# pyprob/pyprob

Hardware: NVIDIA H100
Metric: ic_train_traces_per_sec (higher is better)
Workload: dtype f32

## Files before the change

### pyprob_b200/csrc/net_tc.inc

```
extern unsigned long long* g_trace;
extern int g_trace_launch;

namespace {

inline int64_t img_floats(int64_t rows, int64_t cols) {
  return ((rows + 127) / 128) * ((cols + 31) / 32) * tc::kTileFloats;
}

__global__ void __launch_bounds__(256) k_pack_table(const float* __restrict__ arena, const PackEntry* __restrict__ tab,
                                                     int n_entries, float* __restrict__ wimg) {
  int tile = blockIdx.x;
  int lo = 0, hi = n_entries - 1;
  while (lo < hi) {
    int mid = (lo + hi + 1) >> 1;
    if (tab[mid].tile_start <= tile) lo = mid; else hi = mid - 1;
  }
  const PackEntry e = tab[lo];
  const int rt = tile - e.tile_start;
  const float* src = arena + e.src_off;
  for (int q = threadIdx.x + blockIdx.y * blockDim.x; q < 128 * e.kb * 8; q += blockDim.x * gridDim.y) {
    int c16 = q & 7, t = q >> 3;
    int cb = t % e.kb, r = t / e.kb;
    int row = rt * 128 + r, k0 = cb * 32 + c16 * 4;
    float h[4], l[4];
// ... 65 lines not shown
    gemm::Phase& ph = phases.back();
    if (p.M <= 0 || p.N <= 0 || p.K <= 0) return;
    p.tiles_m = (p.M + 127) / 128;
    p.tiles_n = (p.N + 127) / 128;
    p.tile_start = ph.tiles;
    if (p.k_splits < 1) p.k_splits = 1;
    ph.tiles += p.tiles_m * p.tiles_n * p.k_splits;
    ph.count += 1;
    probs.push_back(p);
  }
};

inline tcg::Operand op_k(const float* hi, const float* lo, int kb, int row0, int col0) {
  tcg::Operand o; o.hi = hi; o.lo = lo; o.k_rows = nullptr; o.kb = kb; o.mn = 0; o.row0 = row0; o.col0 = col0; return o;
}
inline tcg::Operand op_mn(const float* hi, const float* lo, int kb, int row0, int col0, const int* k_rows = nullptr) {
  tcg::Operand o; o.hi = hi; o.lo = lo; o.k_rows = k_rows; o.kb = kb; o.mn = 1; o.row0 = row0; o.col0 = col0; return o;
}
inline tcg::Problem TP0() { tcg::Problem p; memset(&p, 0, sizeof(p)); return p; }
inline tcg::Operand wk(const ppb_net* net, const WImg& w) { return op_k(net->wimg + w.k_hi, net->wimg + w.k_lo, w.kb, 0, 0); }
inline tcg::Operand wmn(const ppb_net* net, const WImg& w) { return op_mn(net->wimg + w.mn_hi, net->wimg + w.mn_lo, w.kb, 0, 0); }

template <bool X3, int EPI>
int launch_tc(const gemm::Phase& ph, const tcg::Problem* dev, cudaStream_t st, unsigned long long* tr) {
  static bool attr_set = false;
  if (!attr_set) {
    PPB_CUDA(cudaFuncSetAttribute(tcg::k_grouped<X3, EPI>, cudaFuncAttributeMaxDynamicSharedMemorySize, (int)tcg::smem_bytes()));
    attr_set = true;
  }
  if (ppb_persistent_enabled() && ph.tiles > PPB_NUM_SMS && tr == nullptr) {
    static bool attr_p = false;
    if (!attr_p) {
      PPB_CUDA(cudaFuncSetAttribute(tcp::k_grouped_persistent<X3, EPI>, cudaFuncAttributeMaxDynamicSharedMemorySize,
                                    (int)tcp::smem_bytes()));
      attr_p = true;
    }
    PPB_CUDA(ppb_launch(tcp::k_grouped_persistent<X3, EPI>, dim3(PPB_NUM_SMS), dim3(tcg::kThreads), tcp::smem_bytes(), st, 1, 0,
                        dev + ph.first, ph.count, ph.tiles));
    return PPB_OK;
  }
  PPB_CUDA(ppb_launch(tcg::k_grouped<X3, EPI>, dim3((unsigned)ph.tiles), dim3(tcg::kThreads), tcg::smem_bytes(), st, 1, 0,
                      dev + ph.first, ph.count, tr));
  return PPB_OK;
}

int run_tc_phase(const gemm::Phase& ph, const tcg::Problem* dev, int precision, cudaStream_t st, int epi,
                 const TcBuilder* bl_for_prof = nullptr) {
  if (ph.count == 0) return PPB_OK;
  cudaEvent_t e0;
  int rc2 = prof_begin(bl_for_prof != nullptr, st, e0); if (rc2) return rc2;
  unsigned long long* tr = nullptr;
  if (g_trace && g_trace_launch < 256) { tr = g_trace + 16 * g_trace_launch; ++g_trace_launch; }
  const bool x3 = precision == PPB_PREC_TF32X3;
  if (epi == 0) rc2 = x3 ? launch_tc<true, 0>(ph, dev, st, tr) : launch_tc<false, 0>(ph, dev, st, tr);
  else if (epi == 1) rc2 = x3 ? launch_tc<true, 1>(ph, dev, st, tr) : launch_tc<false, 1>(ph, dev, st, tr);
  else rc2 = x3 ? launch_tc<true, 2>(ph, dev, st, tr) : launch_tc<false, 2>(ph, dev, st, tr);
  if (rc2) return rc2;
  PPB_LAUNCH_CHECK();
  return e0 ? prof_end(e0, st, phase_flops(bl_for_prof->probs, ph)) : PPB_OK;
}

inline int pick_cluster(int tiles, int min_kc, bool spread_epilogue = false) {
  int cs = 1;
  while (cs < 8 && tiles * cs * 2 <= PPB_NUM_SMS && (spread_epilogue || min_kc / (cs * 2) >= 2)) cs *= 2;
  return cs;
}

template <bool X3, int CS, int EPI, typename RE = tcc::NoRowEpi>
int launch_cluster_tc(const gemm::Phase& ph, const tcg::Problem* dev, cudaStream_t st, const RE& re = RE()) {
  static bool attr_set = false;
  if (!attr_set) {
    PPB_CUDA(cudaFuncSetAttribute(tcc::k_cluster<X3, CS, EPI, RE>, cudaFuncAttributeMaxDynamicSharedMemorySize,
                                  (int)tcc::smem_bytes()));
    attr_set = true;
  }
  unsigned long long* tr = nullptr;
  if (g_trace && g_trace_launch < 256) { tr = g_trace + 16 * g_trace_launch; ++g_trace_launch; }
  PPB_CUDA(tcc::launch_cluster(tcc::k_cluster<X3, CS, EPI, RE>, ph.tiles * CS, CS, tcc::smem_bytes(), st, dev + ph.first,
                               ph.count, tr, re));
// ... 284 lines not shown

int check_tc(const ppb_net* net, const ppb_batch* b) {
  PPB_CHECK_ARG(b->row_align == 128, "the tensor-core path needs a batch encoded with row_align = 128");
  PPB_CHECK_ARG(net->wimg != nullptr, "weight images not built (ppb_net_set_tables)");
  PPB_CHECK_ARG(net->desc.lstm_dim % 32 == 0, "tensor-core path: lstm_dim must be a multiple of 32");
  PPB_CHECK_ARG(b->step_addr_host && b->step_row0_host && b->step_nrows_host && b->step_t_host && b->step_prev_row0_host,
                "missing per-step host arrays");
  return PPB_OK;
}

void add_head_fwd(TcBuilder& tb, const ppb_net* net, const float* arena, const ppb_batch* b, const Ws& w, const TcWs& t,
                  const HImg& x, int kx, const int* x_row0, int& ph_h1, int& ph_h2) {
  const int NS = b->n_steps, dhkb = (net->dh_pad + 31) / 32;
  ph_h1 = (int)tb.phases.size();
  tb.begin();
  for (int s = 0; s < NS; ++s) {
    int aid = b->step_addr_host[s];
    const ppb_addr_desc& a = net->addrs[aid];
    tcg::Problem p = TP0();
    p.a = op_k(x.k_hi, x.k_lo, (int)x.kb, x_row0[s], 0);
    p.b = wk(net, net->w1[aid]);
    p.M = pad128(b->step_nrows_host[s]); p.N = a.head_hidden; p.K = kx;
    p.m_valid = b->step_nrows_host[s];
    p.flags = tcg::kRelu | tcg::kZeroInvalid;
    p.bias = arena + a.b1_off;
    p.o_k_hi = t.hid.k_hi; p.o_k_lo = t.hid.k_lo; p.o_mn_hi = t.hid.mn_hi; p.o_mn_lo = t.hid.mn_lo;
    p.o_kb = dhkb; p.o_row0 = b->step_row0_host[s]; p.o_col0 = 0;
    tb.add(p);
  }
  ph_h2 = (int)tb.phases.size();
  tb.begin();
  for (int s = 0; s < NS; ++s) {
    int aid = b->step_addr_host[s];
    const ppb_addr_desc& a = net->addrs[aid];
    tcg::Problem p = TP0();
    p.a = op_k(t.hid.k_hi, t.hid.k_lo, dhkb, b->step_row0_host[s], 0);
    p.b = wk(net, net->w2[aid]);
    p.M = pad128(b->step_nrows_host[s]); p.N = a.head_out; p.K = a.head_hidden;
    p.bias = arena + a.b2_off;
    p.c = w.out_raw + (int64_t)b->step_row0_host[s] * net->out_pad; p.ldc = net->out_pad;
    p.o_row0 = b->step_row0_host[s];
    tb.add(p);
  }
}

int run_head_nll(ppb_net* net, const ppb_batch* b, const Ws& w, const TcWs& t, const TcBuilder& tb, int ph_h2, int precision,
                 float* loss_out, int32_t* status_out, float* row_lp_out, int want_grad, cudaStream_t st) {
  Dims d = dims_of(b);
  NllArgs na;
  na.addrs = net->d_addrs; na.row_step = b->row_step; na.step_addr = b->step_addr;
  na.values = b->values; na.prior0 = b->prior0; na.prior1 = b->prior1; na.row_trace = b->row_trace;
  na.K = net->desc.mixture_k; na.inv_batch = 1.0f / (float)d.B;
  na.row_lp = row_lp_out ? row_lp_out : w.row_lp; na.d_out = want_grad ? w.d_out : nullptr; na.out_pad = net->out_pad;
  na.dimg = want_grad ? t.d_out : HImg();
  int out_max = 0;
  for (int s = 0; s < d.NS; ++s) out_max = net->addrs[b->step_addr_host[s]].head_out > out_max ? net->addrs[b->step_addr_host[s]].head_out : out_max;
  const int cs_h2 = phase_cluster(tb.phases[ph_h2], tb, true);
  if (cs_h2 > 1 && out_max <= 128) {
    NllRowEpi re;
    re.A = na; re.loss_acc = w.loss_acc; re.loss_out = loss_out; re.status_out = status_out;
    return run_tc_phase_cluster<3>(cs_h2, tb.phases[ph_h2], t.probs, precision, st, re);
  }
  int rc = run_tc_phase_auto(tb.phases[ph_h2], t.probs, precision, st, 0, tb); if (rc) return rc;
  PPB_CUDA(ppb_launch(k_head_nll, dim3(ew_grid((int64_t)d.R * 32, 256)), dim3(256), 0, st, 1, 0, (const float*)w.out_raw, na, d.R,
                      w.loss_acc, loss_out, status_out));
  PPB_LAUNCH_CHECK();
  return PPB_OK;
}

void add_head_dhid(TcBuilder& tb, const ppb_net* net, const ppb_batch* b, const Ws& w, const TcWs& t) {
  const int dhkb = (net->dh_pad + 31) / 32, okb = (net->out_pad + 31) / 32;
  tb.begin();
  for (int s = 0; s < b->n_steps; ++s) {
    int aid = b->step_addr_host[s];
    const ppb_addr_desc& a = net->addrs[aid];
    tcg::Problem p = TP0();
    p.a = op_k(t.d_out.k_hi, t.d_out.k_lo, okb, b->step_row0_host[s], 0);
    p.b = wmn(net, net->w2[aid]);
    p.M = pad128(b->step_nrows_host[s]); p.N = a.head_hidden; p.K = a.head_out;
    p.flags = tcg::kMaskImg;
    p.mask_hi = t.hid.k_hi;
    p.c = w.d_hid + (int64_t)b->step_row0_host[s] * net->dh_pad; p.ldc = net->dh_pad;
    p.o_k_hi = t.d_hid.k_hi; p.o_k_lo = t.d_hid.k_lo; p.o_mn_hi = t.d_hid.mn_hi; p.o_mn_lo = t.d_hid.mn_lo;
    p.o_kb = dhkb; p.o_row0 = b->step_row0_host[s]; p.o_col0 = 0;
    tb.add(p);
  }
}

struct HeadChunks {
  std::vector<std::vector<int>> rows;
  std::vector<int> off, x_off;
};
HeadChunks head_chunks(const ppb_net* net, const ppb_batch* b, const int* x_row0, TcBuilder& tb) {
  HeadChunks h;
  const size_t na = net->addrs.size();
  h.rows.assign(na, std::vector<int>());
  std::vector<std::vector<int>> xr(na);
  for (int s = 0; s < b->n_steps; ++s) {
    int r0 = b->step_row0_host[s], np = pad128(b->step_nrows_host[s]);
    for (int q = 0; q < np; q += 32) {
      h.rows[b->step_addr_host[s]].push_back(r0 + q);
      if (x_row0) xr[b->step_addr_host[s]].push_back(x_row0[s] + q);
    }
// ... 63 lines not shown

int tc_loss_forward(ppb_net* net, const float* arena, const ppb_batch* b, void* workspace, int precision,
                    float* loss_out, int32_t* status_out, float* row_lp_out, int want_grad, cudaStream_t st) {
  int rc = check_tc(net, b);
  if (rc) return rc;
  const ppb_net_desc& D = net->desc;
  Dims d = dims_of(b);
  Ws w = carve(net, d, workspace);
  TcWs t = carve_tc(net, d, (char*)workspace + simt_region_bytes(net, d));
  const int H = D.lstm_dim, H4 = 4 * H, E = D.obs_dim, S = D.sample_dim, I = net->I;
  const int C2 = 2 * (D.type_dim + D.addr_dim);

  TcBuilder tb;
  ObsStep os;
  rc = obs_plan_fwd(net, arena, b, w, t.obs, t.obs_emb, tb, os, st);
  if (rc) return rc;
  const int ph_pobs = (int)tb.phases.size();
  tb.begin();
  {
    tcg::Problem p = TP0();
    p.a = op_k(t.obs_emb.k_hi, t.obs_emb.k_lo, (int)t.obs_emb.kb, 0, 0);
    p.b = wk(net, net->w_ihE);
    p.M = d.B; p.N = H4; p.K = E;
    p.c = w.p_obs; p.ldc = H4;
    tb.add(p);
  }
  std::vector<int> ph_rec(d.T, -1);
  {
    int st0 = 0;
    for (int tt = 0; tt < d.T; ++tt) {
      int st1 = st0;
      while (st1 < d.NS && b->step_t_host[st1] == tt) ++st1;
      if (tt > 0) {
        ph_rec[tt] = (int)tb.phases.size();
        tb.begin();
        for (int s = st0; s < st1; ++s) {
          tcg::Problem p = TP0();
          p.a = op_k(t.h.k_hi, t.h.k_lo, (int)t.h.kb, b->step_prev_row0_host[s], 0);
          p.b = wk(net, net->w_hh);
          p.M = pad128(b->step_nrows_host[s]); p.N = H4; p.K = H;
          p.c = w.gates + (int64_t)b->step_row0_host[s] * H4; p.ldc = H4;
          tb.add(p);
        }
      }
      st0 = st1;
    }
// ... 64 lines not shown
  rc = stream_after(net, st, s2); if (rc) return rc;
  PPB_CUDA(cudaMemsetAsync(w.loss_acc, 0, 256, s1));
  k_pack_table<<<dim3(d.T > 1 ? net->pack_tiles : net->pack_tiles_no_hh, 8), 256, 0, s2>>>(arena, net->d_pack,
                                                                                         (int)net->pack.size(), net->wimg);
  PPB_LAUNCH_CHECK();
  if (fused_cell) {
    tcl::k_pack_whh_interleaved<<<dim3(H / 32, 8), 256, 0, s2>>>(arena + D.w_hh_off, H, net->whh_il,
                                                                 net->whh_il + net->whh_il_floats);
    PPB_LAUNCH_CHECK();
  }
  k_step_embed<<<ew_grid((int64_t)d.NS * C2), 256, 0, s1>>>(arena, net->d_addrs, net->d_type_off, b->step_addr,
                                                            b->step_prev_addr, d.NS, D.type_dim, D.addr_dim, w.emb_cat);
  PPB_LAUNCH_CHECK();
  k_pstep_fwd<<<ew_grid((int64_t)d.NS * H4 * 32), 256, 0, s1>>>(w.emb_cat, arena + D.w_ih_off, arena + D.b_ih_off,
                                                                arena + D.b_hh_off, d.NS, H4, I, E + S, C2, w.p_step);
  PPB_LAUNCH_CHECK();
  if (d.T > 1) {
    k_wsmp_transpose<<<ew_grid(S * H4), 256, 0, s1>>>(arena + D.w_ih_off, I, E, S, H4, w.w_smp_t);
    PPB_LAUNCH_CHECK();
    k_smp_embed<<<ew_grid((int64_t)d.R * S), 256, 0, s1>>>(arena, net->d_addrs, b->row_step, b->step_prev_addr,
                                                           b->row_prev, b->values, d.R, S, w.smp_emb);
    PPB_LAUNCH_CHECK();
  }
  rc = obs_fwd(net, arena, b, w, t.obs, t.obs_emb, tb, t.probs, os, precision, st, s2); if (rc) return rc;
  rc = run_tc_phase_auto(tb.phases[ph_pobs], t.probs, precision, st, 0, tb, true); if (rc) return rc;
  rc = stream_after(net, s1, st); if (rc) return rc;
  for (int tt = 0; tt < d.T; ++tt) {
    int r0 = b->row_off_host[tt], n = b->row_off_host[tt + 1] - r0;
    if (tt > 0 && fused_cell) {
      if (lphase[tt].count == 0) continue;
      const tcl::Step* dsteps = (const tcl::Step*)net->d_lstm_steps;
      const bool x3 = precision == PPB_PREC_TF32X3;
      const int cs = pick_cluster(lphase[tt].tiles, H / 32);
      cudaEvent_t e0;
      rc = prof_begin(true, st, e0); if (rc) return rc;
      if (cs >= 4) rc = x3 ? launch_lstm_cluster<true, 4>(lphase[tt], dsteps, S, st) : launch_lstm_cluster<false, 4>(lphase[tt], dsteps, S, st);
      else if (cs == 2) rc = x3 ? launch_lstm_cluster<true, 2>(lphase[tt], dsteps, S, st) : launch_lstm_cluster<false, 2>(lphase[tt], dsteps, S, st);
      else rc = x3 ? launch_lstm_step<true>(lphase[tt], dsteps, st) : launch_lstm_step<false>(lphase[tt], dsteps, st);
      if (rc) return rc;
      PPB_LAUNCH_CHECK();
      rc = prof_end(e0, st, 2.0 * (double)lphase[tt].tiles * 128.0 * 128.0 * H); if (rc) return rc;
      continue;
    }
    if (tt > 0) { rc = run_tc_phase(tb.phases[ph_rec[tt]], t.probs, precision, st, 0, &tb); if (rc) return rc; }
    PPB_CUDA(ppb_launch(k_cell_fwd, dim3(ew_grid((int64_t)n * H)), dim3(256), 0, st, 1, 0, w.gates, w.p_obs, w.p_step, w.w_smp_t, w.smp_emb, b->row_step,
                                                       b->row_prev, b->row_trace, w.c, w.h, t.h, r0, n, H, S, tt));
// ... 28 lines not shown
  std::vector<int> hh_a, hh_b;
  for (int s = 0; s < d.NS; ++s) {
    int r0 = b->step_row0_host[s], np = pad128(b->step_nrows_host[s]);
    for (int q = 0; q < np; q += 32)
      if (b->step_t_host[s] > 0) { hh_a.push_back(r0 + q); hh_b.push_back(b->step_prev_row0_host[s] + q); }
  }
  const int hh_a_off = (int)tb.ints.size();
  tb.ints.insert(tb.ints.end(), hh_a.begin(), hh_a.end());
  const int hh_b_off = (int)tb.ints.size();
  tb.ints.insert(tb.ints.end(), hh_b.begin(), hh_b.end());
  PPB_CHECK_ARG((int64_t)tb.ints.size() <= t.max_ints, "chunk list overflow");

  const int ph_dhid = 0;
  add_head_dhid(tb, net, b, w, t);
  const int ph_hw = (int)tb.phases.size();
  tb.begin();
  for (int s = 0; s < d.NS; ++s) {
    int aid = b->step_addr_host[s];
    const ppb_addr_desc& a = net->addrs[aid];
    tcg::Problem p = TP0();
    p.a = op_k(t.d_hid.k_hi, t.d_hid.k_lo, dhkb, b->step_row0_host[s], 0);
    p.b = wmn(net, net->w1[aid]);
    p.M = pad128(b->step_nrows_host[s]); p.N = H; p.K = a.head_hidden;
    p.c = w.dh + (int64_t)b->step_row0_host[s] * H; p.ldc = H;
    p.o_row0 = b->step_row0_host[s];
    tb.add(p);
  }
  const int ph_headw = (int)tb.phases.size();
  add_head_weight_grads(tb, net, grad, t, hc, t.h, H);
  std::vector<int> ph_rec(d.T, -1);
  {
    int st1 = d.NS;
    for (int tt = d.T - 1; tt >= 1; --tt) {
      int st0 = st1;
      while (st0 > 0 && b->step_t_host[st0 - 1] == tt) --st0;
      ph_rec[tt] = (int)tb.phases.size();
      tb.begin();
      for (int s = st0; s < st1; ++s) {
        tcg::Problem p = TP0();
        p.a = op_k(t.dgates.k_hi, t.dgates.k_lo, gkb, b->step_row0_host[s], 0);
        p.b = wmn(net, net->w_hh);
        p.M = pad128(b->step_nrows_host[s]); p.N = H; p.K = H4;
        p.c = w.dh_rec + (int64_t)b->step_prev_row0_host[s] * H; p.ldc = H;
        tb.add(p);
      }
      {
// ... 16 lines not shown
  const int ph_lstm_w = (int)tb.phases.size();
  tb.begin();
  if (!hh_a.empty()) {
    tcg::Problem p = TP0();
    p.a = op_mn(t.dgates.mn_hi, t.dgates.mn_lo, gkb, 0, 0, t.ints + hh_a_off);
    p.b = op_mn(t.h.mn_hi, t.h.mn_lo, hkb, 0, 0, t.ints + hh_b_off);
    p.M = H4; p.N = H; p.K = 32 * (int)hh_a.size();
    p.c = grad + D.w_hh_off; p.ldc = H; p.flags = tcg::kAccumulate;
    p.k_splits = pick_splits(p.M, p.N, p.K);
    tb.add(p);
  }
  {
    tcg::Problem p = TP0();
    p.a = op_mn(t.dpobs.mn_hi, t.dpobs.mn_lo, gkb, 0, 0);
    p.b = op_mn(t.obs_emb.mn_hi, t.obs_emb.mn_lo, (int)t.obs_emb.kb, 0, 0);
    p.M = H4; p.N = E; p.K = pad128(d.B);
    p.c = grad + D.w_ih_off; p.ldc = I; p.flags = tcg::kAccumulate;
    p.k_splits = pick_splits(p.M, p.N, p.K);
    tb.add(p);
    tcg::Problem q = TP0();
    q.a = op_k(t.dpobs.k_hi, t.dpobs.k_lo, gkb, 0, 0);
    q.b = wmn(net, net->w_ihE);
    q.M = d.B; q.N = E; q.K = H4;
    q.c = w.d_obs_emb; q.ldc = E;
    q.k_splits = pick_splits(q.M, q.N, q.K);
    tb.add(q);
  }
  ObsStep os;
  rc = obs_plan_bwd(net, arena, grad, b, w, t.obs, tb, os, st);
  if (rc) return rc;
  PPB_CHECK_ARG((int64_t)tb.probs.size() <= t.max_probs / 2, "tensor-core problem list overflow");
  tcg::Problem* tprobs = t.probs + t.max_probs / 2;
  rc = upload_cached(net, 3, tb.probs.data(), tb.probs.size() * sizeof(tcg::Problem), tprobs, st);
  if (rc) return rc;
  rc = upload_cached(net, 4, tb.ints.data(), tb.ints.size() * sizeof(int), t.ints, st);
  if (rc) return rc;

  cudaStream_t s1 = net->side[0], s2 = net->side[1];
  if (d.T > 1) PPB_CUDA(cudaMemsetAsync(w.dh_rec, 0, (size_t)b->row_off_host[d.T - 1] * H * sizeof(float), st));
  PPB_CUDA(cudaMemsetAsync(w.d_pstep, 0, (size_t)((const char*)(w.d_obs_emb + (int64_t)d.B * E) - (const char*)w.d_pstep), st));
  rc = run_tc_phase_auto(tb.phases[ph_dhid], tprobs, precision, st, 2, tb); if (rc) return rc;
  const bool dpobs_fused = (d.B & 127) == 0 && t.dgates.k_hi != nullptr;
  bool dpobs_packed = false;
  const int cs_cell = (d.T == 1 && dpobs_fused) ? phase_cluster(tb.phases[ph_hw], tb, true) : 1;
  if (cs_cell > 1) {
    CellBwdT1Epi re;
    re.gates = w.gates; re.c = w.c; re.row_trace = b->row_trace; re.dgates = dgates; re.pimg = t.dpobs; re.H = H;
    rc = run_tc_phase_cluster<4>(cs_cell, tb.phases[ph_hw], tprobs, precision, st, re); if (rc) return rc;
    dpobs_packed = true;
  } else {
    rc = run_tc_phase_auto(tb.phases[ph_hw], tprobs, precision, st, 0, tb); if (rc) return rc;
    const HImg gimg = d.T > 1 ? t.dgates : HImg();
    float* const dc = d.T > 1 ? w.dc : nullptr;
    for (int tt = d.T - 1; tt >= 0; --tt) {
      int r0 = b->row_off_host[tt], n = b->row_off_host[tt + 1] - r0;
      if (tt + 1 < d.T) { rc = run_tc_phase(tb.phases[ph_rec[tt + 1]], tprobs, precision, st, 1, &tb); if (rc) return rc; }
      if (tt == 0 && dpobs_fused) {
        PPB_CUDA(ppb_launch(k_cell_bwd<true>, dim3(ew_grid((int64_t)n * H)), dim3(256), 0, st, 1, 0, w.gates, w.c, w.dh, w.dh_rec,
                            dc, dgates, w.d_pobs, b->row_prev, b->row_next, b->row_trace, gimg, r0, n, H, tt, t.dpobs));
        dpobs_packed = true;
      } else {
        PPB_CUDA(ppb_launch(k_cell_bwd<false>, dim3(ew_grid((int64_t)n * H)), dim3(256), 0, st, 1, 0, w.gates, w.c, w.dh, w.dh_rec,
                            dc, dgates, w.d_pobs, b->row_prev, b->row_next, b->row_trace, gimg, r0, n, H, tt, HImg()));
      }
      PPB_LAUNCH_CHECK();
    }
  }
  rc = stream_after(net, st, s1); if (rc) return rc;
  rc = run_tc_phase(tb.phases[ph_headw], tprobs, precision, s1, 1); if (rc) return rc;
  rc = launch_head_bias_grad(net, b, w, grad, s1); if (rc) return rc;
  rc = stream_after(net, st, s2); if (rc) return rc;
  const bool one_pass = S <= 4 && H4 <= 2048;
  int max_rows = 0;
  for (int s = 0; s < d.NS; ++s) max_rows = b->step_nrows_host[s] > max_rows ? b->step_nrows_host[s] : max_rows;
  if (one_pass) {
    int slab = (d.R + 2 * PPB_NUM_SMS - 1) / (2 * PPB_NUM_SMS);
    slab = slab < 4 ? 4 : (slab > kRedSlab ? kRedSlab : slab);
    const dim3 g((max_rows + slab - 1) / slab, d.NS);
    const float* wt = d.T > 1 ? w.w_smp_t : w.p_step;
    if (H4 <= 1024)
      k_dgates_reduce<4><<<g, 256, 0, s2>>>(dgates, wt, w.smp_emb, b->values, b->step_prev_addr, b->step_row0, b->step_nrows,
                                            b->row_prev, net->d_addrs, H4, S, I, E, w.d_pstep, grad, D.w_ih_off, slab);
    else
      k_dgates_reduce<8><<<g, 256, 0, s2>>>(dgates, wt, w.smp_emb, b->values, b->step_prev_addr, b->step_row0, b->step_nrows,
                                            b->row_prev, net->d_addrs, H4, S, I, E, w.d_pstep, grad, D.w_ih_off, slab);
    PPB_LAUNCH_CHECK();
  } else {
    dim3 g((H4 + 31) / 32, d.NS);
    k_step_colsum<<<g, 256, 0, s2>>>(dgates, b->step_row0, b->step_nrows, H4, w.d_pstep);
    PPB_LAUNCH_CHECK();
  }
  {
// ... 33 lines not shown
```

### pyprob_b200/csrc/tc_cluster.cuh

```cuda
#pragma once
#include "tc_grouped.cuh"
#include "tc_lstm.cuh"

namespace tcc {

using namespace tc;

constexpr int kPitch = 128;
constexpr int kPartFloats = 128 * kPitch;
static_assert(kPartFloats * 4 <= 2 * tcg::kStages * kTileBytes, "partial tile must fit in the A stages");

__device__ __forceinline__ uint32_t cluster_ctarank() {
  uint32_t r;
  asm volatile("mov.u32 %0, %%cluster_ctarank;" : "=r"(r));
  return r;
}
__device__ __forceinline__ void cluster_sync_all() {
  asm volatile("barrier.cluster.arrive.release.aligned;" ::: "memory");
  asm volatile("barrier.cluster.wait.acquire.aligned;" ::: "memory");
}
__device__ __forceinline__ uint32_t map_to_rank(uint32_t local_smem_addr, uint32_t rank) {
  uint32_t ra;
  asm volatile("mapa.shared::cluster.u32 %0, %1, %2;" : "=r"(ra) : "r"(local_smem_addr), "r"(rank));
  return ra;
// ... 4 lines not shown
  return v;
}

struct __align__(1024) Smem {
  float a_hi[tcg::kStages][kTileFloats];
  float a_lo[tcg::kStages][kTileFloats];
  float b_hi[tcg::kStages][kTileFloats];
  float b_lo[tcg::kStages][kTileFloats];
  uint64_t full[tcg::kStages];
  uint64_t empty[tcg::kStages];
  union { tcg::Problem prob; tcl::Step step; };
};
inline size_t smem_bytes() { return sizeof(Smem) + 1024; }

#define TCC_TRACE(slot)                                                                                   \
  do {                                                                                                    \
    if (trace && blockIdx.x == 0) {                                                                       \
      unsigned long long _t;                                                                              \
      asm volatile("mov.u64 %0, %%globaltimer;" : "=l"(_t));                                              \
      trace[slot] = _t;                                                                                   \
    }                                                                                                     \
  } while (0)

template <bool X3>
__device__ __forceinline__ void mainloop_and_park(Smem& sm, const tcg::Operand& A, const tcg::Operand& B, int mt, int nt,
                                                  int c0, int c1, int warp, int lane,
                                                  unsigned long long* trace = nullptr, int b_prefetched = 0) {
  const tcg::Ring R{sm.a_hi[0], sm.a_lo[0], sm.b_hi[0], sm.b_lo[0], kTileFloats, tcg::kStages, sm.full, sm.empty};
  if (warp == tcg::kProducerWarp) {
    if (lane == 0) {
      const uint32_t bytes = (tcg::stage_bytes(A, mt) + tcg::stage_bytes(B, nt)) * (X3 ? 2u : 1u);
      for (int c = c0; c < c1; ++c) {
        int s = (c - c0) % tcg::kStages;
        uint32_t ph = ((c - c0) / tcg::kStages) & 1;
        mbar_wait(&sm.empty[s], ph ^ 1);
        const bool b_there = c - c0 < b_prefetched;
        if (!b_there) mbar_expect_tx(&sm.full[s], bytes);
        tcg::load_operand(A, mt, c, sm.a_hi[s], sm.a_lo[s], X3, &sm.full[s]);
        if (!b_there) tcg::load_operand(B, nt, c, sm.b_hi[s], sm.b_lo[s], X3, &sm.full[s]);
      }
    }
  } else {
    float acc[32];
    tcg::mma_mainloop<X3>(R, 0, c1 - c0, A.mn != 0, B.mn != 0, warp, lane, acc);
    if (threadIdx.x == 0) TCC_TRACE(3);
    float* part = reinterpret_cast<float*>(sm.a_hi);
    tcg::consumer_sync();
    if (threadIdx.x == 64) TCC_TRACE(4);
    tcg::store_acc(acc, warp, lane, [&](int r, int c) {
      return part + r * kPitch + (c & ~31) + ((((c >> 2) & 7) ^ (r & 7)) << 2) + (c & 3);
    });
  }
  cluster_sync_all();
  if (threadIdx.x == 64) TCC_TRACE(7);
}

template <int CS>
__device__ __forceinline__ void reduce_row(const Smem& sm, int row, int lane, float (&v)[4]) {
  const uint32_t local = smem_u32(reinterpret_cast<const float*>(sm.a_hi) + row * kPitch + ((((lane >> 2) ^ (row & 7))) << 2) +
                                  (lane & 3));
#pragma unroll
  for (int g = 0; g < 4; ++g) v[g] = 0.0f;
#pragma unroll
  for (int s = 0; s < CS; ++s) {
    const uint32_t base = map_to_rank(local, (uint32_t)s);
#pragma unroll
    for (int g = 0; g < 4; ++g) v[g] += ld_cluster(base + g * 32 * 4);
  }
}

__device__ __forceinline__ void common_setup(Smem& sm, int warp, int lane, bool pdl_wait = true) {
  if (warp == tcg::kProducerWarp && lane == 0) {
    for (int s = 0; s < tcg::kStages; ++s) { mbar_init(&sm.full[s], 1); mbar_init(&sm.empty[s], tcg::kEpiWarps); }
    fence_barrier_init();
  }
  __syncthreads();
  ppb_pdl_trigger();
  if (pdl_wait) ppb_pdl_wait();
}

struct NoRowEpi {};
template <typename RE, int EPI> struct RowInOf { struct type {}; };
template <typename RE> struct RowInOf<RE, 3> { using type = typename RE::RowIn; };
template <bool X3, int CS, int EPI, typename RE = NoRowEpi>
__global__ void __launch_bounds__(tcg::kThreads, 1) k_cluster(const tcg::Problem* __restrict__ probs, int n_probs,
                                                                 unsigned long long* __restrict__ trace, const RE re) {
  if (threadIdx.x == 0) TCC_TRACE(0);
  extern __shared__ uint8_t smem_raw[];
  Smem& sm = *reinterpret_cast<Smem*>((reinterpret_cast<uintptr_t>(smem_raw) + 1023) & ~(uintptr_t)1023);
  const int warp = threadIdx.x >> 5, lane = threadIdx.x & 31;
  const int tile = blockIdx.x / CS;
  const int split = (int)cluster_ctarank();
  int lo_i = 0, hi_i = n_probs - 1;
  while (lo_i < hi_i) {
    int mid = (lo_i + hi_i + 1) >> 1;
    if (probs[mid].tile_start <= tile) lo_i = mid; else hi_i = mid - 1;
  }
  for (int i = threadIdx.x; i < (int)(sizeof(tcg::Problem) / 4); i += blockDim.x)
    reinterpret_cast<uint32_t*>(&sm.prob)[i] = reinterpret_cast<const uint32_t*>(probs + lo_i)[i];
  __syncthreads();
  const tcg::Problem& P = sm.prob;
  const int local = tile - P.tile_start;
  const int mt = local / P.tiles_n, nt = local % P.tiles_n;
  const int KC = (P.K + 31) / 32;
  const int c0 = (int)((int64_t)KC * split / CS), c1 = (int)((int64_t)KC * (split + 1) / CS);
  common_setup(sm, warp, lane);
  if (threadIdx.x == 0) TCC_TRACE(1);
  constexpr int kRowsPerCta = 128 / CS, kRowsPerWarp = kRowsPerCta / tcg::kEpiWarps;
  typename RowInOf<RE, EPI>::type rin[kRowsPerWarp];
  if constexpr (EPI == 3) {
    if (warp < tcg::kEpiWarps) {
#pragma unroll
      for (int rr = 0; rr < kRowsPerWarp; ++rr)
        rin[rr] = re.load(P.o_row0 + mt * 128 + split * kRowsPerCta + warp * kRowsPerWarp + rr);
    }
  }
  mainloop_and_park<X3>(sm, P.a, P.b, mt, nt, c0, c1, warp, lane, trace);

  if constexpr (EPI == 3) {
    typename RE::State rs{};
    if (warp < tcg::kEpiWarps) {
      const int pM = P.M, pN = P.N;
      const int64_t orow0 = P.o_row0;
      float bias[4];
#pragma unroll
      for (int g = 0; g < 4; ++g) bias[g] = (P.bias && g * 32 + lane < pN) ? __ldg(P.bias + g * 32 + lane) : 0.0f;
      float r_x[kRowsPerWarp][4];
#pragma unroll
      for (int rr = 0; rr < kRowsPerWarp; ++rr) {
        float v[4];
        reduce_row<CS>(sm, split * kRowsPerCta + warp * kRowsPerWarp + rr, lane, v);
#pragma unroll
        for (int g = 0; g < 4; ++g) r_x[rr][g] = g * 32 + lane < pN ? v[g] + bias[g] : 0.0f;
      }
      float* const xrow = sm.b_hi[0] + warp * 128;
#pragma unroll
      for (int rr = 0; rr < kRowsPerWarp; ++rr) {
        const int m = mt * 128 + split * kRowsPerCta + warp * kRowsPerWarp + rr;
        if (m >= pM) continue;
#pragma unroll
// ... 101 lines not shown
template <bool X3, int CS, int SMAX>
__global__ void __launch_bounds__(tcg::kThreads, 1) k_lstm_cluster(const tcl::Step* __restrict__ steps, int n_steps,
                                                                      unsigned long long* __restrict__ trace) {
  if (threadIdx.x == 0) TCC_TRACE(0);
  extern __shared__ uint8_t smem_raw[];
  Smem& sm = *reinterpret_cast<Smem*>((reinterpret_cast<uintptr_t>(smem_raw) + 1023) & ~(uintptr_t)1023);
  const int warp = threadIdx.x >> 5, lane = threadIdx.x & 31;
  const int tile = blockIdx.x / CS;
  const int split = (int)cluster_ctarank();
  int lo_i = 0, hi_i = n_steps - 1;
  while (lo_i < hi_i) {
    int mid = (lo_i + hi_i + 1) >> 1;
    if (steps[mid].tile_start <= tile) lo_i = mid; else hi_i = mid - 1;
  }
  for (int i = threadIdx.x; i < (int)(sizeof(tcl::Step) / 4); i += blockDim.x)
    reinterpret_cast<uint32_t*>(&sm.step)[i] = reinterpret_cast<const uint32_t*>(steps + lo_i)[i];
  __syncthreads();
  const tcl::Step& P = sm.step;
  const tcl::CellIO& io = P.io;
  const int local = tile - P.tile_start;
  const int mt = local / P.tiles_n, nt = local % P.tiles_n;
  const int KC = (io.H + 31) / 32;
  const int c0 = (int)((int64_t)KC * split / CS), c1 = (int)((int64_t)KC * (split + 1) / CS);
  common_setup(sm, warp, lane, false);
  if (threadIdx.x == 0) TCC_TRACE(1);
  int b_pre = 0;
  if (warp == tcg::kProducerWarp && lane == 0) {
    const uint32_t bytes = (tcg::stage_bytes(P.a, mt) + tcg::stage_bytes(P.b, nt)) * (X3 ? 2u : 1u);
    b_pre = (c1 - c0) < tcg::kStages ? (c1 - c0) : tcg::kStages;
    for (int i = 0; i < b_pre; ++i) {
      mbar_expect_tx(&sm.full[i], bytes);
      tcg::load_operand(P.b, nt, c0 + i, sm.b_hi[i], sm.b_lo[i], X3, &sm.full[i]);
    }
  }
  ppb_pdl_wait();
  constexpr int kRowsPerCta = 128 / CS, kRowsPerWarp = kRowsPerCta / tcg::kEpiWarps;
  int m_tr[kRowsPerWarp], m_st[kRowsPerWarp], m_rp[kRowsPerWarp];
  if (warp < tcg::kEpiWarps) {
#pragma unroll
    for (int rr = 0; rr < kRowsPerWarp; ++rr) {
      const int64_t row = (int64_t)P.row0 + mt * 128 + split * kRowsPerCta + warp * kRowsPerWarp + rr;
      m_tr[rr] = __ldg(io.row_trace + row);
      m_st[rr] = __ldg(io.row_step + row);
      m_rp[rr] = (int)__ldg(io.row_prev + row);
    }
  }
  mainloop_and_park<X3>(sm, P.a, P.b, mt, nt, c0, c1, warp, lane, trace, b_pre);

  if (warp < tcg::kEpiWarps) {
    const int ew = warp;
    const int H = io.H, H4 = 4 * io.H, S = io.S;
    const int u = nt * 32 + lane;
    float wsmp[4][SMAX];
#pragma unroll
    for (int g = 0; g < 4; ++g)
#pragma unroll
      for (int s = 0; s < SMAX; ++s) wsmp[g][s] = (s < S) ? __ldg(io.w_smp_t + (int64_t)s * H4 + g * H + u) : 0.0f;
// ... 81 lines not shown
```

### pyprob_b200/csrc/tc_grouped.cuh

```cuda
#pragma once
#include "common.cuh"
#include "tc.cuh"

namespace tcg {

using namespace tc;

__device__ __forceinline__ void st_global(float* p, float v) { asm volatile("st.global.f32 [%0], %1;" ::"l"(p), "f"(v) : "memory"); }
__device__ __forceinline__ void red_add_global(float* p, float v) { asm volatile("red.global.add.f32 [%0], %1;" ::"l"(p), "f"(v) : "memory"); }
__device__ __forceinline__ float ld_global(const float* p) { float v; asm volatile("ld.global.f32 %0, [%1];" : "=f"(v) : "l"(p)); return v; }

enum : int {
  kRelu = 1,
  kAccumulate = 2,
  kMaskImg = 4,
  kZeroInvalid = 8,
};

struct Operand {
  const float* hi;
  const float* lo;
  const int* k_rows;
  int kb;
  int mn;
  int row0, col0;
};

struct Problem {
  Operand a, b;
  int M, N, K;
  int m_valid;
  int flags;
  float* c;
  int64_t ldc;
  const float* bias;
  float* o_k_hi; float* o_k_lo;
  float* o_mn_hi; float* o_mn_lo;
  const float* mask_hi;
  int o_kb;
// ... 117 lines not shown
        wgmma_tf32_m64n64k8(d, al + 2 * ks, bh + 2 * ks);
        wgmma_tf32_m64n64k8(d, ah + 2 * ks, bl + 2 * ks);
      }
      wgmma_tf32_m64n64k8(d, ah + 2 * ks, bh + 2 * ks);
    }
    wgmma_commit();
    wgmma_wait0();
#pragma unroll
    for (int j = 0; j < 32; ++j) acc[j] += d[j];
    __syncwarp();
    if (lane == 0) mbar_arrive(&R.empty[s]);
  }
}

template <class At>
__device__ __forceinline__ void store_acc(const float (&acc)[32], int warp, int lane, At at) {
  const int r0 = ((warp >> 2) & 1) * 64 + (warp & 3) * 16 + (lane >> 2), c0 = (warp >> 3) * 64 + 2 * (lane & 3);
#pragma unroll
  for (int i = 0; i < 8; ++i)
#pragma unroll
    for (int j = 0; j < 4; ++j) *at(r0 + 8 * (j >> 1), c0 + 8 * i + (j & 1)) = acc[4 * i + j];
}

template <bool X3, bool KTAB = false>
__device__ __forceinline__ void produce(const Ring& R, const Operand& A, const Operand& B, int mt, int nt, int c0, int n,
                                        uint32_t kc0) {
  const uint32_t bytes = (stage_bytes(A, mt) + stage_bytes(B, nt)) * (X3 ? 2u : 1u);
  for (int i = 0; i < n; ++i) {
    const uint32_t kc = kc0 + (uint32_t)i;
    const int s = (int)(kc % (uint32_t)R.stages);
    const uint32_t ph = (kc / (uint32_t)R.stages) & 1;
    mbar_wait(&R.empty[s], ph ^ 1);
    mbar_expect_tx(&R.full[s], bytes);
    load_operand<KTAB>(A, mt, c0 + i, R.a_hi + s * R.stride, R.a_lo + s * R.stride, X3, &R.full[s]);
    load_operand(B, nt, c0 + i, R.b_hi + s * R.stride, R.b_lo + s * R.stride, X3, &R.full[s]);
  }
}

__device__ __forceinline__ Ring ring_of(Smem& sm) {
  return Ring{sm.a_hi[0], sm.a_lo[0], sm.b_hi[0], sm.b_lo[0], kTileFloats, kStages, sm.full, sm.empty};
}

template <bool X3, int EPI, bool KTAB = false>
__global__ void __launch_bounds__(kThreads, 1) k_grouped(const Problem* __restrict__ probs, int n_probs,
                                                          unsigned long long* __restrict__ trace) {
#define TCG_TRACE(slot)                                                                                   \
  do {                                                                                                    \
    if (trace && blockIdx.x == 0) {                                                                       \
      unsigned long long _t;                                                                              \
      asm volatile("mov.u64 %0, %%globaltimer;" : "=l"(_t));                                              \
      trace[slot] = _t;                                                                                   \
    }                                                                                                     \
  } while (0)
  if (threadIdx.x == 0) TCG_TRACE(0);
  extern __shared__ uint8_t smem_raw[];
  Smem& sm = *reinterpret_cast<Smem*>((reinterpret_cast<uintptr_t>(smem_raw) + 1023) & ~(uintptr_t)1023);
  const int warp = threadIdx.x >> 5, lane = threadIdx.x & 31;
  const int tile = blockIdx.x;
// ... 1 lines not shown
  while (lo_i < hi_i) {
    int mid = (lo_i + hi_i + 1) >> 1;
    if (probs[mid].tile_start <= tile) lo_i = mid; else hi_i = mid - 1;
  }
  for (int i = threadIdx.x; i < (int)(sizeof(Problem) / 4); i += blockDim.x)
    reinterpret_cast<uint32_t*>(&sm.prob)[i] = reinterpret_cast<const uint32_t*>(probs + lo_i)[i];
  __syncthreads();
  const Problem& P = sm.prob;
  const int local = tile - P.tile_start;
  const int tiles_mn = P.tiles_m * P.tiles_n;
  const int split = local / tiles_mn, rem = local % tiles_mn;
  const int mt = rem / P.tiles_n, nt = rem % P.tiles_n;
  const int KC = (P.K + 31) / 32;
  const int nsplit = P.k_splits > 1 ? P.k_splits : 1;
  const int c0 = (int)((int64_t)KC * split / nsplit), c1 = (int)((int64_t)KC * (split + 1) / nsplit);

  if (warp == kProducerWarp && lane == 0) {
    for (int s = 0; s < kStages; ++s) { mbar_init(&sm.full[s], 1); mbar_init(&sm.empty[s], kEpiWarps); }
    fence_barrier_init();
  }
  __syncthreads();
  if (threadIdx.x == 0) TCG_TRACE(1);
  ppb_pdl_trigger();
  ppb_pdl_wait();
  const Ring R = ring_of(sm);

  if (warp == kProducerWarp) {
    if (lane == 0) produce<X3, KTAB>(R, P.a, P.b, mt, nt, c0, c1 - c0, 0);
  } else {
    float acc[32];
    mma_mainloop<X3>(R, 0, c1 - c0, P.a.mn != 0, P.b.mn != 0, warp, lane, acc);
    if (threadIdx.x == 0) TCG_TRACE(3);
    float* const ctile = sm.b_hi[0];
    consumer_sync();
    store_acc(acc, warp, lane, [&](int r, int c) { return ctile + r * kCPitch + c; });
    consumer_sync();
    if (threadIdx.x == 0) TCG_TRACE(4);
    const int q = warp & 3;
    const int cb = warp >> 2;
    const float* stg = ctile + (q * 32) * kCPitch + cb * 32;
    const int m_base = mt * 128 + q * 32;
    const bool do_relu = (P.flags & kRelu) != 0, do_mask = (P.flags & kMaskImg) != 0;
    const int rows = (P.M - m_base) < 32 ? (P.M - m_base) : 32;
    const int valid_rows = (P.flags & kZeroInvalid) ? (P.m_valid - m_base) : 32;
    const float* bias_p = P.bias;
    const float* mask_p = P.mask_hi;
    float* c_p = P.c;
    float* ok_hi = P.o_k_hi; float* ok_lo = P.o_k_lo; float* omn_hi = P.o_mn_hi; float* omn_lo = P.o_mn_lo;
    const int64_t ldc = P.ldc, o_kb = P.o_kb, orow0 = (int64_t)P.o_row0 + m_base, ocb0 = P.o_col0 / 32 + nt * 4;
    {
      const int n0 = nt * kBN + cb * 32;
      if (n0 < ((P.N + 31) & ~31) && m_base < P.M) {
// ... 73 lines not shown
```

### pyprob_b200/csrc/tc_persist.cuh

```cuda
#pragma once
#include "tc_grouped.cuh"

namespace tcp {

using namespace tc;

template <bool X3> struct StageCfg { static constexpr int kStages = X3 ? 2 : 4; static constexpr int kFloats = (X3 ? 4 : 2) * kTileFloats; };

constexpr int kMaxStages = 4;
struct __align__(1024) Smem {
  float ring[8 * kTileFloats];
  float ctile[tcg::kCFloats];
  uint64_t full[kMaxStages];
  uint64_t empty[kMaxStages];
};
inline size_t smem_bytes() { return sizeof(Smem) + 1024; }

__device__ __forceinline__ int find_problem(const tcg::Problem* __restrict__ probs, int n_probs, int tile) {
  int lo = 0, hi = n_probs - 1;
  while (lo < hi) {
    const int mid = (lo + hi + 1) >> 1;
    if (probs[mid].tile_start <= tile) lo = mid; else hi = mid - 1;
  }
  return lo;
// ... 7 lines not shown
  const int KC = (P.K + 31) / 32;
  const int nsplit = P.k_splits > 1 ? P.k_splits : 1;
  TileGeom g;
  g.mt = rem / P.tiles_n; g.nt = rem % P.tiles_n;
  g.c0 = (int)((int64_t)KC * split / nsplit); g.c1 = (int)((int64_t)KC * (split + 1) / nsplit);
  return g;
}

template <bool X3, int EPI>
__global__ void __launch_bounds__(tcg::kThreads, 1) k_grouped_persistent(const tcg::Problem* __restrict__ probs, int n_probs,
                                                                          int total_tiles) {
  extern __shared__ uint8_t smem_raw[];
  Smem& sm = *reinterpret_cast<Smem*>((reinterpret_cast<uintptr_t>(smem_raw) + 1023) & ~(uintptr_t)1023);
  const int warp = threadIdx.x >> 5, lane = threadIdx.x & 31;
  constexpr int kStages = StageCfg<X3>::kStages, kStageFloats = StageCfg<X3>::kFloats;
  const tcg::Ring R{sm.ring, sm.ring + 2 * kTileFloats, sm.ring + kTileFloats, sm.ring + 3 * kTileFloats, kStageFloats, kStages,
                    sm.full, sm.empty};
  if (warp == tcg::kProducerWarp && lane == 0) {
    for (int s = 0; s < kStages; ++s) { mbar_init(&sm.full[s], 1); mbar_init(&sm.empty[s], tcg::kEpiWarps); }
    fence_barrier_init();
  }
  __syncthreads();
  ppb_pdl_trigger();
  ppb_pdl_wait();

  if (warp == tcg::kProducerWarp) {
    if (lane == 0) {
      uint32_t kc = 0;
      for (int tile = blockIdx.x; tile < total_tiles; tile += gridDim.x) {
        const tcg::Problem& P = probs[find_problem(probs, n_probs, tile)];
        const TileGeom g = tile_geom(P, tile);
        tcg::produce<X3>(R, P.a, P.b, g.mt, g.nt, g.c0, g.c1 - g.c0, kc);
        kc += (uint32_t)(g.c1 - g.c0);
      }
    }
  } else {
    const int q = warp & 3;
    const int cb = warp >> 2;
    const float* stg = sm.ctile + (q * 32) * tcg::kCPitch + cb * 32;
    uint32_t kc = 0;
    for (int tile = blockIdx.x; tile < total_tiles; tile += gridDim.x) {
      int pi = 0;
      if (lane == 0) pi = find_problem(probs, n_probs, tile);
      pi = __shfl_sync(0xffffffffu, pi, 0);
      const tcg::Problem& P = probs[pi];
      const TileGeom g = tile_geom(P, tile);
      float acc[32];
      tcg::mma_mainloop<X3>(R, kc, g.c1 - g.c0, P.a.mn != 0, P.b.mn != 0, warp, lane, acc);
      kc += (uint32_t)(g.c1 - g.c0);
      tcg::consumer_sync();
      tcg::store_acc(acc, warp, lane, [&](int r, int c) { return sm.ctile + r * tcg::kCPitch + c; });
      tcg::consumer_sync();
      const int pM = P.M, pN = P.N, flags = P.flags;
      const int m_base = g.mt * 128 + q * 32;
      const bool do_relu = (flags & tcg::kRelu) != 0, do_mask = (flags & tcg::kMaskImg) != 0;
      const int rows = (pM - m_base) < 32 ? (pM - m_base) : 32;
// ... 60 lines not shown
```

Before: 1.594 million.

## Prefetch weight operand tiles before PDL wait in grouped and cluster GEMMs

Adds a kBPrefetch flag so GEMM kernels whose B operand is a static weight issue the first pipeline stages of B loads before waiting on the previous kernel via programmatic dependent launch. This is applied to grouped, persistent and cluster kernels, which overlaps weight loading with the prior kernel's tail. Gradient-buffer memsets move from the backward stream to an earlier side stream in forward, and the head weight-grad phase on the side stream no longer uses PDL. The risk is extra code in the producer path and correctness only if B is truly independent of the preceding kernel.

After: 1.592 million (median of 6 runs). No clear change (-0.1%).

```diff
diff --git a/pyprob_b200/csrc/net_tc.inc b/pyprob_b200/csrc/net_tc.inc
--- a/pyprob_b200/csrc/net_tc.inc
+++ b/pyprob_b200/csrc/net_tc.inc
@@ -111,7 +111,7 @@
 inline tcg::Operand wmn(const ppb_net* net, const WImg& w) { return op_mn(net->wimg + w.mn_hi, net->wimg + w.mn_lo, w.kb, 0, 0); }
 
 template <bool X3, int EPI>
-int launch_tc(const gemm::Phase& ph, const tcg::Problem* dev, cudaStream_t st, unsigned long long* tr) {
+int launch_tc(const gemm::Phase& ph, const tcg::Problem* dev, cudaStream_t st, unsigned long long* tr, bool pdl) {
   static bool attr_set = false;
   if (!attr_set) {
     PPB_CUDA(cudaFuncSetAttribute(tcg::k_grouped<X3, EPI>, cudaFuncAttributeMaxDynamicSharedMemorySize, (int)tcg::smem_bytes()));
@@ -124,26 +124,26 @@
                                     (int)tcp::smem_bytes()));
       attr_p = true;
     }
-    PPB_CUDA(ppb_launch(tcp::k_grouped_persistent<X3, EPI>, dim3(PPB_NUM_SMS), dim3(tcg::kThreads), tcp::smem_bytes(), st, 1, 0,
+    PPB_CUDA(ppb_launch(tcp::k_grouped_persistent<X3, EPI>, dim3(PPB_NUM_SMS), dim3(tcg::kThreads), tcp::smem_bytes(), st, pdl, 0,
                         dev + ph.first, ph.count, ph.tiles));
     return PPB_OK;
   }
-  PPB_CUDA(ppb_launch(tcg::k_grouped<X3, EPI>, dim3((unsigned)ph.tiles), dim3(tcg::kThreads), tcg::smem_bytes(), st, 1, 0,
+  PPB_CUDA(ppb_launch(tcg::k_grouped<X3, EPI>, dim3((unsigned)ph.tiles), dim3(tcg::kThreads), tcg::smem_bytes(), st, pdl, 0,
                       dev + ph.first, ph.count, tr));
   return PPB_OK;
 }
 
 int run_tc_phase(const gemm::Phase& ph, const tcg::Problem* dev, int precision, cudaStream_t st, int epi,
-                 const TcBuilder* bl_for_prof = nullptr) {
+                 const TcBuilder* bl_for_prof = nullptr, bool pdl = true) {
   if (ph.count == 0) return PPB_OK;
   cudaEvent_t e0;
   int rc2 = prof_begin(bl_for_prof != nullptr, st, e0); if (rc2) return rc2;
   unsigned long long* tr = nullptr;
   if (g_trace && g_trace_launch < 256) { tr = g_trace + 16 * g_trace_launch; ++g_trace_launch; }
   const bool x3 = precision == PPB_PREC_TF32X3;
-  if (epi == 0) rc2 = x3 ? launch_tc<true, 0>(ph, dev, st, tr) : launch_tc<false, 0>(ph, dev, st, tr);
-  else if (epi == 1) rc2 = x3 ? launch_tc<true, 1>(ph, dev, st, tr) : launch_tc<false, 1>(ph, dev, st, tr);
-  else rc2 = x3 ? launch_tc<true, 2>(ph, dev, st, tr) : launch_tc<false, 2>(ph, dev, st, tr);
+  if (epi == 0) rc2 = x3 ? launch_tc<true, 0>(ph, dev, st, tr, pdl) : launch_tc<false, 0>(ph, dev, st, tr, pdl);
+  else if (epi == 1) rc2 = x3 ? launch_tc<true, 1>(ph, dev, st, tr, pdl) : launch_tc<false, 1>(ph, dev, st, tr, pdl);
+  else rc2 = x3 ? launch_tc<true, 2>(ph, dev, st, tr, pdl) : launch_tc<false, 2>(ph, dev, st, tr, pdl);
   if (rc2) return rc2;
   PPB_LAUNCH_CHECK();
   return e0 ? prof_end(e0, st, phase_flops(bl_for_prof->probs, ph)) : PPB_OK;
@@ -474,7 +474,7 @@
     p.b = wk(net, net->w1[aid]);
     p.M = pad128(b->step_nrows_host[s]); p.N = a.head_hidden; p.K = kx;
     p.m_valid = b->step_nrows_host[s];
-    p.flags = tcg::kRelu | tcg::kZeroInvalid;
+    p.flags = tcg::kRelu | tcg::kZeroInvalid | tcg::kBPrefetch;
     p.bias = arena + a.b1_off;
     p.o_k_hi = t.hid.k_hi; p.o_k_lo = t.hid.k_lo; p.o_mn_hi = t.hid.mn_hi; p.o_mn_lo = t.hid.mn_lo;
     p.o_kb = dhkb; p.o_row0 = b->step_row0_host[s]; p.o_col0 = 0;
@@ -489,6 +489,7 @@
     p.a = op_k(t.hid.k_hi, t.hid.k_lo, dhkb, b->step_row0_host[s], 0);
     p.b = wk(net, net->w2[aid]);
     p.M = pad128(b->step_nrows_host[s]); p.N = a.head_out; p.K = a.head_hidden;
+    p.flags = tcg::kBPrefetch;
     p.bias = arena + a.b2_off;
     p.c = w.out_raw + (int64_t)b->step_row0_host[s] * net->out_pad; p.ldc = net->out_pad;
     p.o_row0 = b->step_row0_host[s];
@@ -530,7 +531,7 @@
     p.a = op_k(t.d_out.k_hi, t.d_out.k_lo, okb, b->step_row0_host[s], 0);
     p.b = wmn(net, net->w2[aid]);
     p.M = pad128(b->step_nrows_host[s]); p.N = a.head_hidden; p.K = a.head_out;
-    p.flags = tcg::kMaskImg;
+    p.flags = tcg::kMaskImg | tcg::kBPrefetch;
     p.mask_hi = t.hid.k_hi;
     p.c = w.d_hid + (int64_t)b->step_row0_host[s] * net->dh_pad; p.ldc = net->dh_pad;
     p.o_k_hi = t.d_hid.k_hi; p.o_k_lo = t.d_hid.k_lo; p.o_mn_hi = t.d_hid.mn_hi; p.o_mn_lo = t.d_hid.mn_lo;
@@ -640,6 +641,7 @@
     p.a = op_k(t.obs_emb.k_hi, t.obs_emb.k_lo, (int)t.obs_emb.kb, 0, 0);
     p.b = wk(net, net->w_ihE);
     p.M = d.B; p.N = H4; p.K = E;
+    p.flags = tcg::kBPrefetch;
     p.c = w.p_obs; p.ldc = H4;
     tb.add(p);
   }
@@ -750,6 +752,8 @@
                                                            b->row_prev, b->values, d.R, S, w.smp_emb);
     PPB_LAUNCH_CHECK();
   }
+  if (d.T > 1) PPB_CUDA(cudaMemsetAsync(w.dh_rec, 0, (size_t)b->row_off_host[d.T - 1] * H * sizeof(float), s1));
+  PPB_CUDA(cudaMemsetAsync(w.d_pstep, 0, (size_t)((const char*)(w.d_obs_emb + (int64_t)d.B * E) - (const char*)w.d_pstep), s1));
   rc = obs_fwd(net, arena, b, w, t.obs, t.obs_emb, tb, t.probs, os, precision, st, s2); if (rc) return rc;
   rc = run_tc_phase_auto(tb.phases[ph_pobs], t.probs, precision, st, 0, tb, true); if (rc) return rc;
   rc = stream_after(net, s1, st); if (rc) return rc;
@@ -824,6 +828,7 @@
     p.a = op_k(t.d_hid.k_hi, t.d_hid.k_lo, dhkb, b->step_row0_host[s], 0);
     p.b = wmn(net, net->w1[aid]);
     p.M = pad128(b->step_nrows_host[s]); p.N = H; p.K = a.head_hidden;
+    p.flags = tcg::kBPrefetch;
     p.c = w.dh + (int64_t)b->step_row0_host[s] * H; p.ldc = H;
     p.o_row0 = b->step_row0_host[s];
     tb.add(p);
@@ -886,6 +891,7 @@
     q.a = op_k(t.dpobs.k_hi, t.dpobs.k_lo, gkb, 0, 0);
     q.b = wmn(net, net->w_ihE);
     q.M = d.B; q.N = E; q.K = H4;
+    q.flags = tcg::kBPrefetch;
     q.c = w.d_obs_emb; q.ldc = E;
     q.k_splits = pick_splits(q.M, q.N, q.K);
     tb.add(q);
@@ -901,8 +907,6 @@
   if (rc) return rc;
 
   cudaStream_t s1 = net->side[0], s2 = net->side[1];
-  if (d.T > 1) PPB_CUDA(cudaMemsetAsync(w.dh_rec, 0, (size_t)b->row_off_host[d.T - 1] * H * sizeof(float), st));
-  PPB_CUDA(cudaMemsetAsync(w.d_pstep, 0, (size_t)((const char*)(w.d_obs_emb + (int64_t)d.B * E) - (const char*)w.d_pstep), st));
   rc = run_tc_phase_auto(tb.phases[ph_dhid], tprobs, precision, st, 2, tb); if (rc) return rc;
   const bool dpobs_fused = (d.B & 127) == 0 && t.dgates.k_hi != nullptr;
   bool dpobs_packed = false;
@@ -931,7 +935,7 @@
     }
   }
   rc = stream_after(net, st, s1); if (rc) return rc;
-  rc = run_tc_phase(tb.phases[ph_headw], tprobs, precision, s1, 1); if (rc) return rc;
+  rc = run_tc_phase(tb.phases[ph_headw], tprobs, precision, s1, 1, nullptr, false); if (rc) return rc;
   rc = launch_head_bias_grad(net, b, w, grad, s1); if (rc) return rc;
   rc = stream_after(net, st, s2); if (rc) return rc;
   const bool one_pass = S <= 4 && H4 <= 2048;
diff --git a/pyprob_b200/csrc/tc_cluster.cuh b/pyprob_b200/csrc/tc_cluster.cuh
--- a/pyprob_b200/csrc/tc_cluster.cuh
+++ b/pyprob_b200/csrc/tc_cluster.cuh
@@ -50,25 +50,19 @@
     }                                                                                                     \
   } while (0)
 
+__device__ __forceinline__ tcg::Ring ring_of(Smem& sm) {
+  return tcg::Ring{sm.a_hi[0], sm.a_lo[0], sm.b_hi[0], sm.b_lo[0], kTileFloats, tcg::kStages, sm.full, sm.empty};
+}
+
 template <bool X3>
 __device__ __forceinline__ void mainloop_and_park(Smem& sm, const tcg::Operand& A, const tcg::Operand& B, int mt, int nt,
                                                   int c0, int c1, int warp, int lane,
                                                   unsigned long long* trace = nullptr, int b_prefetched = 0) {
-  const tcg::Ring R{sm.a_hi[0], sm.a_lo[0], sm.b_hi[0], sm.b_lo[0], kTileFloats, tcg::kStages, sm.full, sm.empty};
+  const tcg::Ring R = ring_of(sm);
   if (warp == tcg::kProducerWarp) {
-    if (lane == 0) {
-      const uint32_t bytes = (tcg::stage_bytes(A, mt) + tcg::stage_bytes(B, nt)) * (X3 ? 2u : 1u);
-      for (int c = c0; c < c1; ++c) {
-        int s = (c - c0) % tcg::kStages;
-        uint32_t ph = ((c - c0) / tcg::kStages) & 1;
-        mbar_wait(&sm.empty[s], ph ^ 1);
-        const bool b_there = c - c0 < b_prefetched;
-        if (!b_there) mbar_expect_tx(&sm.full[s], bytes);
-        tcg::load_operand(A, mt, c, sm.a_hi[s], sm.a_lo[s], X3, &sm.full[s]);
-        if (!b_there) tcg::load_operand(B, nt, c, sm.b_hi[s], sm.b_lo[s], X3, &sm.full[s]);
-      }
-    }
+    if (lane == 0) tcg::produce<X3>(R, A, B, mt, nt, c0, c1 - c0, 0, b_prefetched);
   } else {
+    if (trace && threadIdx.x == 0 && blockIdx.x == 0 && c1 > c0) { mbar_wait(&sm.full[0], 0); TCC_TRACE(2); }
     float acc[32];
     tcg::mma_mainloop<X3>(R, 0, c1 - c0, A.mn != 0, B.mn != 0, warp, lane, acc);
     if (threadIdx.x == 0) TCC_TRACE(3);
@@ -97,14 +91,13 @@
   }
 }
 
-__device__ __forceinline__ void common_setup(Smem& sm, int warp, int lane, bool pdl_wait = true) {
+__device__ __forceinline__ void common_setup(Smem& sm, int warp, int lane) {
   if (warp == tcg::kProducerWarp && lane == 0) {
     for (int s = 0; s < tcg::kStages; ++s) { mbar_init(&sm.full[s], 1); mbar_init(&sm.empty[s], tcg::kEpiWarps); }
     fence_barrier_init();
   }
   __syncthreads();
   ppb_pdl_trigger();
-  if (pdl_wait) ppb_pdl_wait();
 }
 
 struct NoRowEpi {};
@@ -133,7 +126,11 @@
   const int KC = (P.K + 31) / 32;
   const int c0 = (int)((int64_t)KC * split / CS), c1 = (int)((int64_t)KC * (split + 1) / CS);
   common_setup(sm, warp, lane);
-  if (threadIdx.x == 0) TCC_TRACE(1);
+  int b_pre = 0;
+  if ((P.flags & tcg::kBPrefetch) && warp == tcg::kProducerWarp && lane == 0) {
+    b_pre = tcg::prefetch_b<X3>(ring_of(sm), P.a, P.b, mt, nt, c0, c1 - c0);
+    TCC_TRACE(15);
+  }
   constexpr int kRowsPerCta = 128 / CS, kRowsPerWarp = kRowsPerCta / tcg::kEpiWarps;
   typename RowInOf<RE, EPI>::type rin[kRowsPerWarp];
   if constexpr (EPI == 3) {
@@ -143,7 +140,9 @@
         rin[rr] = re.load(P.o_row0 + mt * 128 + split * kRowsPerCta + warp * kRowsPerWarp + rr);
     }
   }
-  mainloop_and_park<X3>(sm, P.a, P.b, mt, nt, c0, c1, warp, lane, trace);
+  ppb_pdl_wait();
+  if (threadIdx.x == 0) TCC_TRACE(1);
+  mainloop_and_park<X3>(sm, P.a, P.b, mt, nt, c0, c1, warp, lane, trace, b_pre);
 
   if constexpr (EPI == 3) {
     typename RE::State rs{};
@@ -291,17 +290,10 @@
   const int mt = local / P.tiles_n, nt = local % P.tiles_n;
   const int KC = (io.H + 31) / 32;
   const int c0 = (int)((int64_t)KC * split / CS), c1 = (int)((int64_t)KC * (split + 1) / CS);
-  common_setup(sm, warp, lane, false);
+  common_setup(sm, warp, lane);
   if (threadIdx.x == 0) TCC_TRACE(1);
   int b_pre = 0;
-  if (warp == tcg::kProducerWarp && lane == 0) {
-    const uint32_t bytes = (tcg::stage_bytes(P.a, mt) + tcg::stage_bytes(P.b, nt)) * (X3 ? 2u : 1u);
-    b_pre = (c1 - c0) < tcg::kStages ? (c1 - c0) : tcg::kStages;
-    for (int i = 0; i < b_pre; ++i) {
-      mbar_expect_tx(&sm.full[i], bytes);
-      tcg::load_operand(P.b, nt, c0 + i, sm.b_hi[i], sm.b_lo[i], X3, &sm.full[i]);
-    }
-  }
+  if (warp == tcg::kProducerWarp && lane == 0) b_pre = tcg::prefetch_b<X3>(ring_of(sm), P.a, P.b, mt, nt, c0, c1 - c0);
   ppb_pdl_wait();
   constexpr int kRowsPerCta = 128 / CS, kRowsPerWarp = kRowsPerCta / tcg::kEpiWarps;
   int m_tr[kRowsPerWarp], m_st[kRowsPerWarp], m_rp[kRowsPerWarp];
diff --git a/pyprob_b200/csrc/tc_grouped.cuh b/pyprob_b200/csrc/tc_grouped.cuh
--- a/pyprob_b200/csrc/tc_grouped.cuh
+++ b/pyprob_b200/csrc/tc_grouped.cuh
@@ -15,6 +15,7 @@
   kAccumulate = 2,
   kMaskImg = 4,
   kZeroInvalid = 8,
+  kBPrefetch = 16,
 };
 
 struct Operand {
@@ -178,18 +179,30 @@
     for (int j = 0; j < 4; ++j) *at(r0 + 8 * (j >> 1), c0 + 8 * i + (j & 1)) = acc[4 * i + j];
 }
 
+template <bool X3>
+__device__ __forceinline__ int prefetch_b(const Ring& R, const Operand& A, const Operand& B, int mt, int nt, int c0, int n) {
+  const uint32_t bytes = (stage_bytes(A, mt) + stage_bytes(B, nt)) * (X3 ? 2u : 1u);
+  const int k = n < R.stages ? n : R.stages;
+  for (int i = 0; i < k; ++i) {
+    mbar_expect_tx(&R.full[i], bytes);
+    load_operand(B, nt, c0 + i, R.b_hi + i * R.stride, R.b_lo + i * R.stride, X3, &R.full[i]);
+  }
+  return k;
+}
+
 template <bool X3, bool KTAB = false>
 __device__ __forceinline__ void produce(const Ring& R, const Operand& A, const Operand& B, int mt, int nt, int c0, int n,
-                                        uint32_t kc0) {
+                                        uint32_t kc0, int b_pre = 0) {
   const uint32_t bytes = (stage_bytes(A, mt) + stage_bytes(B, nt)) * (X3 ? 2u : 1u);
   for (int i = 0; i < n; ++i) {
     const uint32_t kc = kc0 + (uint32_t)i;
     const int s = (int)(kc % (uint32_t)R.stages);
     const uint32_t ph = (kc / (uint32_t)R.stages) & 1;
     mbar_wait(&R.empty[s], ph ^ 1);
-    mbar_expect_tx(&R.full[s], bytes);
+    const bool b_there = i < b_pre;
+    if (!b_there) mbar_expect_tx(&R.full[s], bytes);
     load_operand<KTAB>(A, mt, c0 + i, R.a_hi + s * R.stride, R.a_lo + s * R.stride, X3, &R.full[s]);
-    load_operand(B, nt, c0 + i, R.b_hi + s * R.stride, R.b_lo + s * R.stride, X3, &R.full[s]);
+    if (!b_there) load_operand(B, nt, c0 + i, R.b_hi + s * R.stride, R.b_lo + s * R.stride, X3, &R.full[s]);
   }
 }
 
@@ -237,12 +250,18 @@
   __syncthreads();
   if (threadIdx.x == 0) TCG_TRACE(1);
   ppb_pdl_trigger();
+  const Ring R = ring_of(sm);
+  int b_pre = 0;
+  if ((P.flags & kBPrefetch) && warp == kProducerWarp && lane == 0) {
+    b_pre = prefetch_b<X3>(R, P.a, P.b, mt, nt, c0, c1 - c0);
+    TCG_TRACE(15);
+  }
   ppb_pdl_wait();
-  const Ring R = ring_of(sm);
 
   if (warp == kProducerWarp) {
-    if (lane == 0) produce<X3, KTAB>(R, P.a, P.b, mt, nt, c0, c1 - c0, 0);
+    if (lane == 0) produce<X3, KTAB>(R, P.a, P.b, mt, nt, c0, c1 - c0, 0, b_pre);
   } else {
+    if (trace && threadIdx.x == 0 && blockIdx.x == 0 && c1 > c0) { mbar_wait(&R.full[0], 0); TCG_TRACE(2); }
     float acc[32];
     mma_mainloop<X3>(R, 0, c1 - c0, P.a.mn != 0, P.b.mn != 0, warp, lane, acc);
     if (threadIdx.x == 0) TCG_TRACE(3);
diff --git a/pyprob_b200/csrc/tc_persist.cuh b/pyprob_b200/csrc/tc_persist.cuh
--- a/pyprob_b200/csrc/tc_persist.cuh
+++ b/pyprob_b200/csrc/tc_persist.cuh
@@ -53,6 +53,14 @@
   }
   __syncthreads();
   ppb_pdl_trigger();
+  int b_pre = 0;
+  if (warp == tcg::kProducerWarp && lane == 0 && (int)blockIdx.x < total_tiles) {
+    const tcg::Problem& P = probs[find_problem(probs, n_probs, blockIdx.x)];
+    if (P.flags & tcg::kBPrefetch) {
+      const TileGeom g = tile_geom(P, blockIdx.x);
+      b_pre = tcg::prefetch_b<X3>(R, P.a, P.b, g.mt, g.nt, g.c0, g.c1 - g.c0);
+    }
+  }
   ppb_pdl_wait();
 
   if (warp == tcg::kProducerWarp) {
@@ -61,8 +69,9 @@
       for (int tile = blockIdx.x; tile < total_tiles; tile += gridDim.x) {
         const tcg::Problem& P = probs[find_problem(probs, n_probs, tile)];
         const TileGeom g = tile_geom(P, tile);
-        tcg::produce<X3>(R, P.a, P.b, g.mt, g.nt, g.c0, g.c1 - g.c0, kc);
+        tcg::produce<X3>(R, P.a, P.b, g.mt, g.nt, g.c0, g.c1 - g.c0, kc, b_pre);
         kc += (uint32_t)(g.c1 - g.c0);
+        b_pre = 0;
       }
     }
   } else {
```
